# libshoal/Green-Marl

Hardware: AMD Instinct MI355X
Metric: edges/s (GTEPS) per PageRank iter, RMAT-26 (higher is better)
Workload: dtype f32; 1 GPU; pagerank RMAT-26 (V=67108864, E=1073741824), reference RMAT generator seed 1997 permute=1, d=0.85, fixed iterations; partition=1-D vertex, 1 rank(s), exchange=none, exchange_bytes_per_rank_and_step=0, exchange_packed=False, step_form=single rank, options=15

## Files before the change

green-marl_amd/csrc/gmx_pr_cold.hip:

```cpp
#pragma clang fp contract(off)

#include "gmx_internal.h"

#include <algorithm>
#include <rocprim/rocprim.hpp>

#define PRC_G 32
#define PRC_BLK_GROUPS 16
#define PRC_LDS_BYTES 131072
#define PRC_STAGE_BYTES 2048
#define PRC_LDS_LIMIT 163840
static constexpr int prc_tile_elems(int elem) { return (PRC_LDS_LIMIT - 16 * (PRC_STAGE_BYTES + 64 * elem) - 64) / elem; }
static constexpr int prc_tile_elems_classed(int elem) {
    return (PRC_LDS_LIMIT - 16 * 64 * elem - 64) / elem < 32768 ? (PRC_LDS_LIMIT - 16 * 64 * elem - 64) / elem / 8 * 8 : 32768;
}
#define PRC_THREADS 1024
#define PRC_WAVES (PRC_THREADS / 64)
#define PRC_UNROLL 4
#define PRC_PAD 0xffffu
#define PRC_END 0x8000u
#define PRC_Q1P 0
#define PRC_Q1E 64
#define PRC_Q2 128

// ... 784 lines not shown
            V4 v;
            v.x = s_tile[ids[u].x & 0x7fffu];
            v.y = s_tile[(ids[u].x >> 16) & 0x7fffu];
            v.z = s_tile[ids[u].y & 0x7fffu];
            v.w = s_tile[(ids[u].y >> 16) & 0x7fffu];
            __builtin_nontemporal_store(v, (V4*) (val + o[u]) + (lane & 7));
        }
    }
}

template <typename S, int TILE, bool CLASSED>
__global__ void __launch_bounds__(PRC_THREADS)
pr_cold_tile_kernel(const prc_item1* __restrict__ items, int n_items, unsigned int* __restrict__ queue,
                    const S* __restrict__ contrib, const int32_t* __restrict__ org, int nranks, int64_t span, int64_t slice, int64_t T,
                    const uint16_t* __restrict__ srcl, const int32_t* __restrict__ ob, S* __restrict__ val, unsigned sink_base,
                    unsigned qbase, const int32_t* __restrict__ vst) {
    __shared__ S s_tile[TILE];
    __shared__ S s_stage[PRC_WAVES][CLASSED ? 64 : PRC_STAGE_BYTES / sizeof(S) + 64];
    __shared__ int s_item;
    const int tid = threadIdx.x, lane = tid & 63;
    const int wv = __builtin_amdgcn_readfirstlane(tid >> 6);
    const unsigned sink = sink_base + (blockIdx.x * PRC_WAVES + wv) * 64 + lane;
    int loaded = -1;
    for (;;) {
        __syncthreads();
        if (tid == 0) s_item = (int) (atomicAdd(&queue[CLASSED ? PRC_Q1E : PRC_Q1P], 1u) - qbase);
        __syncthreads();
        const int it = s_item;
        if ((unsigned) it >= (unsigned) n_items) break;
        const prc_item1 d = items[it];
        if (d.tile != loaded) {
            prc_load_tile<S, TILE>(s_tile, d.tile, org, contrib, nranks, span, slice, T);
            loaded = d.tile;
            __syncthreads();
        }
        if constexpr (CLASSED) {
            const int32_t* vs = vst + ((int64_t) d.tile << PRC_CLS_BITS);
            for (int cls = PRC_CL_E1; cls <= PRC_CL_H; cls++) {
                const int32_t lo = max(d.g0, vs[cls]), hi = min(d.g1, vs[cls + 1]);
                if (lo >= hi) continue;
                const prc_item1 seg{d.tile, lo, hi, cls + 1};
                switch (cls) {
                case PRC_CL_E1: prc_class_item<S, PRC_FORM_E1>(seg, s_tile, s_stage[wv], srcl, ob, val, sink, wv, lane); break;
                case PRC_CL_E2: prc_class_item<S, PRC_FORM_E2>(seg, s_tile, s_stage[wv], srcl, ob, val, sink, wv, lane); break;
                case PRC_CL_E4: prc_class_item<S, PRC_FORM_E4>(seg, s_tile, s_stage[wv], srcl, ob, val, sink, wv, lane); break;
                case PRC_CL_E8: prc_class_item<S, PRC_FORM_E8>(seg, s_tile, s_stage[wv], srcl, ob, val, sink, wv, lane); break;
                default: prc_class_item<S, PRC_FORM_H>(seg, s_tile, s_stage[wv], srcl, ob, val, sink, wv, lane); break;
                }
            }
        } else {
            if (d.form == PRC_FORM_PAIR) prc_pair_item<S>(d, s_tile, s_stage[wv], srcl, ob, val, sink, wv, lane);
            else prc_edge_item<S>(d, s_tile, srcl, ob, val, wv, lane);
        }
    }
}

__device__ __forceinline__ unsigned long long prc_fix_hi(double v) { return (unsigned long long) (long long) (v * 0x1p62); }

template <typename S>
__device__ __forceinline__ void prc_finish_row(const pr_cold_fuse& fz, int64_t i, double sum, double& diff_acc) {
    const int32_t od = __builtin_nontemporal_load(fz.outdeg_c + i);
    const int64_t r = __builtin_nontemporal_load(fz.active + i);
    const double old = (double) __builtin_nontemporal_load((const S*) fz.rk_c + i);
    const S vs = (S) (fz.base + fz.d * sum);
    diff_acc += fabs((double) vs - old);
    __builtin_nontemporal_store(vs, (S*) fz.rk_c + i);
    __builtin_nontemporal_store(od > 0 ? (S) ((double) vs / (double) od) : (S) 0, (S*) fz.next_owned + r);
}

template <int THREADS>
__device__ __forceinline__ void prc_block_diff(double diff_acc, double* s_red, double* __restrict__ dst) {
#pragma unroll
    for (int off = 32; off > 0; off >>= 1) diff_acc += __shfl_down(diff_acc, off, 64);
    if ((threadIdx.x & 63) == 0) s_red[threadIdx.x >> 6] = diff_acc;
    __syncthreads();
    if (threadIdx.x == 0) {
        double t = 0.0;
#pragma unroll
        for (int w = 0; w < THREADS / 64; w++) t += s_red[w];
        *dst = t;
    }
}

template <typename S, int BINROWS, int LIMBS, bool FUSE>
__global__ void __launch_bounds__(PRC_THREADS)
pr_cold_accum_kernel(const prc_item2* __restrict__ items, int n_items, unsigned int* __restrict__ queue,
                     const uint16_t* __restrict__ rowl, const S* __restrict__ val, int64_t nactive, double lo_scale,
                     S* __restrict__ cold, unsigned long long* __restrict__ scratch, pr_cold_fuse fz,
                     double* __restrict__ diff_part, unsigned qbase) {
    typedef typename prc_vec4<S>::type V4;
    __shared__ unsigned long long s_acc[LIMBS * BINROWS];
    __shared__ double s_red[PRC_WAVES];
    __shared__ int s_item;
    const int tid = threadIdx.x, lane = tid & 63;
    const int wv = __builtin_amdgcn_readfirstlane(tid >> 6);
    for (;;) {
        __syncthreads();
        if (tid == 0) s_item = (int) (atomicAdd(&queue[PRC_Q2], 1u) - qbase);
#pragma unroll 4
        for (int i = tid; i < LIMBS * BINROWS; i += PRC_THREADS) s_acc[i] = 0ull;
        __syncthreads();
        const int it = s_item;
        if ((unsigned) it >= (unsigned) n_items) break;
        const prc_item2 d = items[it];
        const int npieces = (d.g1 - d.g0 + 7) >> 3;
        for (int base = 0; base < npieces; base += PRC_WAVES * PRC_UNROLL) {
            prc_u32x2 ids[PRC_UNROLL];
            V4 v[PRC_UNROLL];
            bool ok[PRC_UNROLL];
#pragma unroll
            for (int u = 0; u < PRC_UNROLL; u++) {
                const int pc = base + u * PRC_WAVES + wv;
                const int g = d.g0 + pc * 8 + (lane >> 3);
                ok[u] = pc < npieces && g < d.g1;
                if (ok[u]) {
                    const int64_t at = (int64_t) g * (PRC_G / 4) + (lane & 7);
                    ids[u] = __builtin_nontemporal_load((const prc_u32x2*) rowl + at);
                    v[u] = __builtin_nontemporal_load((const V4*) val + at);
                }
            }
#pragma unroll
            for (int u = 0; u < PRC_UNROLL; u++) {
                if (!ok[u]) continue;
                const unsigned r[4] = {ids[u].x & 0xffffu, ids[u].x >> 16, ids[u].y & 0xffffu, ids[u].y >> 16};
                const double x[4] = {(double) v[u].x, (double) v[u].y, (double) v[u].z, (double) v[u].w};
#pragma unroll
                for (int j = 0; j < 4; j++) {
                    if (r[j] == PRC_PAD) continue;
                    PRC_CHECK(r[j] < (unsigned) BINROWS && x[j] >= 0.0 && x[j] <= 1.0);
                    const unsigned long long hi = prc_fix_hi(x[j]);
                    __hip_atomic_fetch_add(&s_acc[r[j]], hi, __ATOMIC_RELAXED, __HIP_MEMORY_SCOPE_WORKGROUP);
                    if (LIMBS > 1) {
                        const double rem = x[j] - (double) (long long) hi * 0x1p-62;
                        const unsigned long long lo = (unsigned long long) (long long) (rem * 0x1p62 * lo_scale);
                        __hip_atomic_fetch_add(&s_acc[BINROWS + r[j]], lo, __ATOMIC_RELAXED, __HIP_MEMORY_SCOPE_WORKGROUP);
                    }
                }
            }
        }
        __syncthreads();
        double diff_acc = 0.0;
        if (d.slot < 0) {
            const int64_t i0 = (int64_t) d.bin * BINROWS;
#pragma unroll 4
            for (int r = tid; r < BINROWS; r += PRC_THREADS) {
                if (i0 + r >= nactive) break;
                double sum = (double) (long long) s_acc[r] * 0x1p-62;
                if (LIMBS > 1) sum += (double) (long long) s_acc[BINROWS + r] * (0x1p-62 / lo_scale);
                if (FUSE) prc_finish_row<S>(fz, i0 + r, sum, diff_acc);
                else __builtin_nontemporal_store((S) sum, cold + i0 + r);
            }
        } else {
            unsigned long long* dst = scratch + (int64_t) d.slot * (LIMBS * BINROWS);
#pragma unroll 4
            for (int i = tid; i < LIMBS * BINROWS; i += PRC_THREADS) dst[i] = s_acc[i];
        }
        if (FUSE) prc_block_diff<PRC_THREADS>(diff_acc, s_red, diff_part + it);
    }
}

template <typename S, int BINROWS, int LIMBS, bool FUSE>
__global__ void __launch_bounds__(1024)
pr_cold_reduce_kernel(const prc_item3* __restrict__ items, int64_t nactive, double lo_scale,
                      const unsigned long long* __restrict__ scratch, S* __restrict__ cold, pr_cold_fuse fz,
                      double* __restrict__ diff_part) {
    __shared__ unsigned long long s_part[LIMBS][16][64];
    const prc_item3 d = items[blockIdx.y];
    const int lane = threadIdx.x & 63, wv = threadIdx.x >> 6;
    const int r = blockIdx.x * 64 + lane;
    const int64_t i0 = (int64_t) d.bin * BINROWS;
    unsigned long long hi = 0, lo = 0;
    const unsigned long long* src = scratch + (int64_t) d.slot0 * (LIMBS * BINROWS) + r;
#pragma unroll 4
    for (int s = wv; s < d.nslots; s += 16) {
        hi += __builtin_nontemporal_load(src + (int64_t) s * (LIMBS * BINROWS));
        if (LIMBS > 1) lo += __builtin_nontemporal_load(src + (int64_t) s * (LIMBS * BINROWS) + BINROWS);
    }
    s_part[0][wv][lane] = hi;
    if (LIMBS > 1) s_part[LIMBS - 1][wv][lane] = lo;
    __syncthreads();
    if (wv == 0 && i0 + r < nactive) {
        hi = 0;
        lo = 0;
#pragma unroll
        for (int w = 0; w < 16; w++) {
            hi += s_part[0][w][lane];
            if (LIMBS > 1) lo += s_part[LIMBS - 1][w][lane];
        }
        double v = (double) (long long) hi * 0x1p-62;
        if (LIMBS > 1) v += (double) (long long) lo * (0x1p-62 / lo_scale);
        if (FUSE) {
            double diff_acc = 0.0;
            prc_finish_row<S>(fz, i0 + r, v, diff_acc);
            s_part[0][0][lane] = (unsigned long long) __double_as_longlong(diff_acc);
        } else cold[i0 + r] = (S) v;
    } else if (FUSE && wv == 0) s_part[0][0][lane] = 0ull;
    if (FUSE && wv == 0) {
        __builtin_amdgcn_wave_barrier();
        __builtin_amdgcn_s_waitcnt(0xc07f);
        __builtin_amdgcn_wave_barrier();
        if (lane == 0) {
            double t = 0.0;
            for (int l = 0; l < 64; l++) t += __longlong_as_double((long long) s_part[0][0][l]);
            diff_part[(int64_t) blockIdx.y * gridDim.x + blockIdx.x] = t;
        }
    }
}

#define PRC_FEW_SLOTS 8
template <typename S, int BINROWS, int LIMBS, bool FUSE>
__global__ void __launch_bounds__(256)
pr_cold_reduce_few_kernel(const prc_item3* __restrict__ items, int64_t nactive, double lo_scale,
                          const unsigned long long* __restrict__ scratch, S* __restrict__ cold, pr_cold_fuse fz,
                          double* __restrict__ diff_part) {
    const prc_item3 d = items[blockIdx.y];
    const int lane = threadIdx.x & 63;
    const int rg = blockIdx.x * 4 + (threadIdx.x >> 6);
    const int r = rg * 64 + lane;
    const int64_t i0 = (int64_t) d.bin * BINROWS;
    unsigned long long hi = 0, lo = 0;
    const unsigned long long* src = scratch + (int64_t) d.slot0 * (LIMBS * BINROWS) + r;
#pragma unroll 4
    for (int s = 0; s < d.nslots; s++) {
        hi += __builtin_nontemporal_load(src + (int64_t) s * (LIMBS * BINROWS));
        if (LIMBS > 1) lo += __builtin_nontemporal_load(src + (int64_t) s * (LIMBS * BINROWS) + BINROWS);
    }
    double diff_acc = 0.0;
    if (i0 + r < nactive) {
        double v = (double) (long long) hi * 0x1p-62;
        if (LIMBS > 1) v += (double) (long long) lo * (0x1p-62 / lo_scale);
        if (FUSE) prc_finish_row<S>(fz, i0 + r, v, diff_acc);
        else cold[i0 + r] = (S) v;
    }
    if (FUSE) {
        double t = 0.0;
        for (int l = 0; l < 64; l++) t += __shfl(diff_acc, l, 64);
        if (lane == 0) diff_part[(int64_t) blockIdx.y * (BINROWS / 64) + rg] = t;
    }
}

// ... 86 lines not shown
    } while (0)
#define PRC_ALLOC(buf, count)                        \
    do {                                             \
        if ((st = (buf).alloc((size_t) (count)))) goto done; \
    } while (0)

static int prc_env_int(const char* name, int dflt) {
    const char* v = getenv(name);
    return v && *v ? atoi(v) : dflt;
}

static hipError_t prc_exscan(const int32_t* in, int32_t* out, int64_t n, wbuf<char>& tmp, hipStream_t s) {
    size_t tb = 0;
    hipError_t e = rocprim::exclusive_scan(nullptr, tb, in, out, 0, (size_t) n, rocprim::plus<int32_t>(), s);
    if (e != hipSuccess) return e;
    if (tmp.n < tb) {
        tmp.release();
        if (tmp.alloc(tb)) return hipErrorOutOfMemory;
    }
    return rocprim::exclusive_scan((void*) tmp.p, tb, in, out, 0, (size_t) n, rocprim::plus<int32_t>(), s);
}

static hipError_t prc_inscan(const int32_t* in, int32_t* out, int64_t n, wbuf<char>& tmp, hipStream_t s) {
    size_t tb = 0;
    hipError_t e = rocprim::inclusive_scan(nullptr, tb, in, out, (size_t) n, rocprim::plus<int32_t>(), s);
    if (e != hipSuccess) return e;
    if (tmp.n < tb) {
        tmp.release();
        if (tmp.alloc(tb)) return hipErrorOutOfMemory;
    }
    return rocprim::inclusive_scan((void*) tmp.p, tb, in, out, (size_t) n, rocprim::plus<int32_t>(), s);
}

int pr_cold_create(const uint64_t* keys, int64_t Ec, const pr_cold_params& prm, hipStream_t s, pr_cold** outp) {
    *outp = nullptr;
    GMX_REQUIRE(prm.elem == 4 || prm.elem == 8, "pr cold: bad element size");
    GMX_REQUIRE(prm.T >= 0 && prm.T < prm.slice, "pr cold: threshold outside the rank range");
    GMX_REQUIRE(Ec < (1LL << 31) - (1LL << 27), "pr cold: %lld edges exceed the int32 stream positions", (long long) Ec);
    pr_cold* c = new pr_cold();
    c->prm = prm;
    c->Ec = Ec;
    const int64_t class_density = prc_env_int("GMX_PR_COLD_CLASS_DENSITY", 1);
    const bool all_classed = class_density == 1;
    c->tile = all_classed ? prc_tile_elems_classed(prm.elem) : prc_tile_elems(prm.elem);
    const int tile_src = c->tile - 1;
    c->limbs = prm.elem == 4 ? 1 : 2;
    c->binrows = PRC_LDS_BYTES / 8 / c->limbs;
    c->ncold = (int64_t) prm.nranks * (prm.slice - prm.T);
    c->ntiles = (c->ncold + tile_src - 1) / tile_src;
    c->nbins = (prm.nactive + c->binrows - 1) / c->binrows;
    if (c->nbins < 1) c->nbins = 1;
    const int tilebits = gmx_bits_for(c->ntiles), binbits = gmx_bits_for(c->nbins), vtbits = tilebits + PRC_CLS_BITS;
    const int64_t nvt = c->ntiles << PRC_CLS_BITS;
    const double pair_min = prc_env_int("GMX_PR_COLD_PAIR_X100", 125) / 100.0;
    int st = GMX_OK;
    gmx_tick tick("cold plan");
    gmx_ws_scope ws;
    wbuf<uint64_t> k1, k2;
    wbuf<int32_t> cflag, cincl, ps, pincl, pstart, plen, ppos, pos, endf, endpre, first, pfirst, groups, c1raw, c1, vtab, delta, counts, id, order2, groups2,
        c2s, c2, tab2, tstat;
    wbuf<uint32_t> ckey, key2, key2s;
    wbuf<uint8_t> mode;
    wbuf<char> tmp;
    uint64_t* sk = nullptr;
    std::vector<int32_t> hts, hvt, hdelta, vstart, h2;
    std::vector<uint8_t> hmode;
    std::vector<prc_item1> v1p, v1e;
    std::vector<prc_item2> v2;
    std::vector<prc_item3> v3;
    int64_t ngroups1 = 0, ngroups2 = 0, nc = 0, np = 0, pair_edges = 0, pair_tiles = 0, class_tiles = 0, class_edges = 0;
    hipDeviceProp_t prop;
    int dev = 0;
    if (vtbits + binbits > 32) {
        gmx_set_error("pr cold: %lld tiles x %lld bins do not fit the sort key", (long long) c->ntiles, (long long) c->nbins);
        st = GMX_ERR_ARG;
        goto done;
    }
    PRC_ALLOC(c->cold, (size_t) (prm.nactive ? prm.nactive : 1) * prm.elem);
    PRC_TRY(hipMemsetAsync(c->cold.p, 0, (size_t) (prm.nactive ? prm.nactive : 1) * prm.elem, s), "memset");
    PRC_ALLOC(c->queue, 3 * 64);
    PRC_TRY(hipMemsetAsync(c->queue.p, 0, 3 * 64 * sizeof(unsigned int), s), "memset");
    (void) hipGetDevice(&dev);
    PRC_TRY(hipGetDeviceProperties(&prop, dev), "hipGetDeviceProperties");
    c->grid = prop.multiProcessorCount;
    if (Ec == 0) {
        PRC_TRY(hipStreamSynchronize(s), "sync");
        *outp = c;
        return GMX_OK;
    }
    {
        PRC_ALLOC(k1, Ec);
        PRC_ALLOC(k2, Ec);
        hipLaunchKernelGGL(prc_keys_kernel, dim3(prc_grid_for(Ec)), dim3(256), 0, s, keys, Ec, prm, tile_src, c->binrows, binbits, k1.p);
        rocprim::double_buffer<uint64_t> db(k1.p, k2.p);
        size_t tb = 0;
        const unsigned end_bit = 32u + (unsigned) binbits + (unsigned) vtbits;
        PRC_TRY(rocprim::radix_sort_keys(nullptr, tb, db, (size_t) Ec, 16u, end_bit, s), "sort size");
        PRC_ALLOC(tmp, tb);
        PRC_TRY(rocprim::radix_sort_keys((void*) tmp.p, tb, db, (size_t) Ec, 16u, end_bit, s), "sort");
        PRC_TRY(hipStreamSynchronize(s), "sort sync");
        sk = db.current();
    }
    tick.mark("keys + main sort");
    PRC_ALLOC(cflag, Ec + 1);
    PRC_ALLOC(cincl, Ec + 1);
    PRC_ALLOC(ps, Ec + 1);
    PRC_ALLOC(pincl, Ec + 1);
    PRC_ALLOC(mode, c->ntiles + 1);
    PRC_ALLOC(tstat, 3 * (c->ntiles + 1));
    hmode.assign((size_t) c->ntiles + 1, PRC_TM_EDGE);
    for (int round = 0; round < 2; round++) {
        hipLaunchKernelGGL(prc_runs_kernel, dim3(prc_grid_for(Ec)), dim3(256), 0, s, (const uint64_t*) sk, Ec,
                           round ? (const uint8_t*) mode.p : (const uint8_t*) nullptr, 32 + binbits + PRC_CLS_BITS, cflag.p, ps.p);
        PRC_TRY(prc_inscan(cflag.p, cincl.p, Ec, tmp, s), "scan");
        PRC_TRY(prc_inscan(ps.p, pincl.p, Ec, tmp, s), "scan");
        {
            int32_t lastc = 0, lastp = 0;
            PRC_TRY(hipMemcpyAsync(&lastc, cincl.p + (Ec - 1), 4, hipMemcpyDeviceToHost, s), "copy");
            PRC_TRY(hipMemcpyAsync(&lastp, pincl.p + (Ec - 1), 4, hipMemcpyDeviceToHost, s), "copy");
            PRC_TRY(hipStreamSynchronize(s), "sync");
            c->ncells = nc = lastc;
            np = lastp;
        }
        if (pstart.n < (size_t) np + 1) { pstart.release(); PRC_ALLOC(pstart, np + 1); }
        hipLaunchKernelGGL(prc_pair_start_kernel, dim3(prc_grid_for(Ec + 1)), dim3(256), 0, s, (const int32_t*) ps.p, (const int32_t*) pincl.p, Ec, np, pstart.p);
        if (round == 1) break;
        hipLaunchKernelGGL(prc_tile_stats_kernel, dim3(prc_grid_for(c->ntiles + 1)), dim3(256), 0, s, (const uint64_t*) sk, Ec,
                           32 + binbits + PRC_CLS_BITS, c->ntiles, (const int32_t*) pincl.p, (const int32_t*) cincl.p, np, nc, tstat.p);
        hts.resize((size_t) 3 * (c->ntiles + 1));
        PRC_TRY(hipMemcpyAsync(hts.data(), tstat.p, sizeof(int32_t) * hts.size(), hipMemcpyDeviceToHost, s), "copy");
        PRC_TRY(hipStreamSynchronize(s), "sync");
        for (int64_t t = 0; t < c->ntiles; t++) {
            const int64_t ne = (int64_t) hts[3 * (t + 1)] - hts[3 * t], npt = (int64_t) hts[3 * (t + 1) + 1] - hts[3 * t + 1],
                          nct = (int64_t) hts[3 * (t + 1) + 2] - hts[3 * t + 2];
            hmode[t] = (npt > 0 && (double) ne >= pair_min * (double) npt) ? PRC_TM_PAIR : PRC_TM_EDGE;
            if (hmode[t] == PRC_TM_PAIR) { pair_edges += ne; pair_tiles++; }
            if (hmode[t] == PRC_TM_PAIR && class_density > 0 && ne >= class_density * nct) { hmode[t] = PRC_TM_CLASSED; class_tiles++; class_edges += ne; }
            else if (hmode[t] == PRC_TM_EDGE && all_classed && ne > 0) { hmode[t] = PRC_TM_SINGLES; class_tiles++; class_edges += ne; }
        }
        PRC_TRY(hipMemcpyAsync(mode.p, hmode.data(), hmode.size(), hipMemcpyHostToDevice, s), "copy");
        if (class_tiles == 0) continue;
        hipLaunchKernelGGL(prc_class_kernel, dim3(prc_grid_for(Ec)), dim3(256), 0, s, sk, Ec, (const int32_t*) pincl.p, (const int32_t*) pstart.p,
                           (const uint8_t*) mode.p, binbits);
        {
            uint64_t* other = sk == k1.p ? k2.p : k1.p;
            rocprim::double_buffer<uint64_t> db(sk, other);
            size_t tb = 0;
            const unsigned b0 = 32u + (unsigned) binbits, b1 = b0 + (unsigned) vtbits;
            PRC_TRY(rocprim::radix_sort_keys(nullptr, tb, db, (size_t) Ec, b0, b1, s), "sort size");
            if (tmp.n < tb) { tmp.release(); PRC_ALLOC(tmp, tb); }
            PRC_TRY(rocprim::radix_sort_keys((void*) tmp.p, tb, db, (size_t) Ec, b0, b1, s), "sort");
            PRC_TRY(hipStreamSynchronize(s), "sort sync");
            sk = db.current();
        }
    }
    if (sk == k1.p) k2.release(); else k1.release();
    tick.mark("runs, classes, class sort");
    ps.release();
    PRC_ALLOC(plen, np + 1);
    PRC_ALLOC(ppos, np + 1);
    hipLaunchKernelGGL(prc_pair_len_kernel, dim3(prc_grid_for(np + 1)), dim3(256), 0, s, (const uint64_t*) sk, (const int32_t*) pstart.p, np, binbits, plen.p);
    PRC_TRY(prc_exscan(plen.p, ppos.p, np + 1, tmp, s), "scan");
    plen.release();
    PRC_ALLOC(first, nc + 1);
    PRC_ALLOC(pfirst, nc + 1);
    PRC_ALLOC(ckey, nc + 1);
    PRC_ALLOC(groups, nc + 1);
// ... 119 lines not shown
    }
    if (prm.deg_by_id) {
        wbuf<int32_t> tmax;
        PRC_ALLOC(tmax, c->ntiles);
        PRC_TRY(hipMemsetAsync(tmax.p, 0, sizeof(int32_t) * (size_t) c->ntiles, s), "memset");
        const int64_t nids = (int64_t) prm.nranks * prm.slice;
        hipLaunchKernelGGL(prc_tile_maxdeg_kernel, dim3(prc_grid_for(nids)), dim3(256), 0, s, prm.deg_by_id, nids, prm.slice, prm.T, tile_src, tmax.p);
        c->tile_maxdeg.assign((size_t) c->ntiles, 0);
        PRC_TRY(hipMemcpyAsync(c->tile_maxdeg.data(), tmax.p, sizeof(int32_t) * (size_t) c->ntiles, hipMemcpyDeviceToHost, s), "copy");
        PRC_TRY(hipStreamSynchronize(s), "sync");
    }
    {
        const int64_t want1 = std::max<int64_t>(ngroups1 / ((int64_t) c->grid * 4), std::min<int64_t>(8192, ngroups1 / ((int64_t) c->grid * 2)));
        const int64_t want2 = ngroups2 / ((int64_t) c->grid * 2);
        const int ch1 = (int) std::min<int64_t>(262144, std::max<int64_t>(PRC_SUPER_GROUPS, prc_env_int("GMX_PR_COLD_CHUNK1", (int) std::min<int64_t>(want1, 32768)))) / PRC_SUPER_GROUPS * PRC_SUPER_GROUPS;
        const int ch2 = (int) std::min<int64_t>(32768, std::max<int64_t>(8, prc_env_int("GMX_PR_COLD_CHUNK", (int) std::min<int64_t>(std::max<int64_t>(want2, 2048), 32768)))) / 8 * 8;
        const int64_t thr2 = (int64_t) ch2 * prc_env_int("GMX_PR_COLD_SPLIT_X100", 300) / 100;
        for (int64_t t = 0; t < c->ntiles; t++) {
            const int64_t v0 = t << PRC_CLS_BITS;
            if (hmode[t] == PRC_TM_CLASSED || hmode[t] == PRC_TM_SINGLES) {
                const int32_t g0 = vstart[v0 + PRC_CL_E1], g1 = vstart[v0 + PRC_CL_H + 1];
                for (int32_t g = g0; g < g1; g += ch1) v1p.push_back({(int32_t) t, g, std::min(g1, g + ch1), PRC_FORM_TILE});
                continue;
            }
            const int32_t graw = hvt[2 * (v0 + 1) + 1] - hvt[2 * v0 + 1];
            if (graw == 0) continue;
            const int32_t g0 = vstart[v0];
            const int form = hmode[t] == PRC_TM_PAIR ? PRC_FORM_PAIR : PRC_FORM_EDGE;
            const int32_t g1 = form == PRC_FORM_PAIR ? vstart[v0 + 1] : g0 + graw;
            for (int32_t g = g0; g < g1; g += ch1) (form == PRC_FORM_EDGE ? v1e : v1p).push_back({(int32_t) t, g, std::min(g1, g + ch1), form});
        }
        PRC_ALLOC(c->vstart, vstart.size());
        PRC_TRY(hipMemcpy(c->vstart.p, vstart.data(), sizeof(int32_t) * vstart.size(), hipMemcpyHostToDevice), "copy");
        int32_t slot = 0;
        c->all_bins = true;
        for (int64_t b = 0; b < c->nbins; b++) {
            const int32_t g0 = h2[b], g1 = h2[b + 1];
            if (g1 <= g0) { c->all_bins = false; continue; }
            if (g1 - g0 <= thr2) { v2.push_back({(int32_t) b, g0, g1, -1}); continue; }
            const int32_t s0 = slot;
            for (int32_t g = g0; g < g1; g += ch2) v2.push_back({(int32_t) b, g, std::min(g1, g + ch2), slot++});
            v3.push_back({(int32_t) b, s0, slot - s0, 0});
        }
        c->n1p = (int64_t) v1p.size();
        c->n1e = (int64_t) v1e.size();
        c->n2 = (int64_t) v2.size();
        c->n3 = (int64_t) v3.size();
        c->nslots = slot;
        PRC_ALLOC(c->it1p, std::max<size_t>(1, v1p.size() + v1e.size()));
        PRC_ALLOC(c->it2, std::max<size_t>(1, v2.size()));
        PRC_ALLOC(c->it3, std::max<size_t>(1, v3.size()));
        PRC_ALLOC(c->scratch, std::max<size_t>(1, (size_t) slot * c->limbs * c->binrows));
        PRC_ALLOC(c->diffp, std::max<size_t>(1, v2.size() + v3.size() * (size_t) (c->binrows / 64)));
        PRC_TRY(hipMemset(c->diffp.p, 0, sizeof(double) * std::max<size_t>(1, v2.size() + v3.size() * (size_t) (c->binrows / 64))), "memset");
        c->h1p.swap(v1p);
        c->h1e.swap(v1e);
        c->h2.swap(v2);
        c->h3.swap(v3);
        if ((st = prc_upload_lists(c, nullptr, nullptr, 1))) goto done;
    }
    PRC_TRY(hipStreamSynchronize(s), "sync");
    tick.mark("tables, work lists");
    if (getenv("GMX_PR_DEBUG")) {
        std::vector<int64_t> bs;
        for (int64_t b = 0; b < c->nbins; b++) bs.push_back(((int64_t) h2[b + 1] - h2[b]) * PRC_G);
        std::sort(bs.begin(), bs.end());
        int64_t over[4] = {0, 0, 0, 0}, lim[4] = {131072, 262144, 524288, 1048576}, sum_over[4] = {0, 0, 0, 0};
        for (int64_t v : bs)
            for (int q = 0; q < 4; q++)
                if (v > lim[q]) { over[q]++; sum_over[q] += v; }
        fprintf(stderr, "gmx pr cold: bin items min %lld median %lld p90 %lld max %lld; bins over 128K/256K/512K/1M items: %lld/%lld/%lld/%lld holding %lld/%lld/%lld/%lld items\n",
                (long long) bs.front(), (long long) bs[bs.size() / 2], (long long) bs[bs.size() * 9 / 10], (long long) bs.back(),
                (long long) over[0], (long long) over[1], (long long) over[2], (long long) over[3], (long long) sum_over[0],
                (long long) sum_over[1], (long long) sum_over[2], (long long) sum_over[3]);
        int64_t cg[1 << PRC_CLS_BITS] = {0};
        for (int64_t v = 0; v < nvt; v++) cg[v & ((1 << PRC_CLS_BITS) - 1)] += (int64_t) vstart[v + 1] - vstart[v];
        fprintf(stderr, "gmx pr cold: T %lld, %lld edges -> %lld entries in %lld cells (%lld tiles x %lld bins); %lld pair tiles with %lld edges, of them %lld "
                "in length classes with %lld edges; groups by class generic/E1/E2/E4/E8/H %lld/%lld/%lld/%lld/%lld/%lld; %lld natural pairs -> %lld item ends -> "
                "%lld items; work items %lld + %lld / %lld / %lld, %lld slots, lo_bits %d\n", (long long) prm.T, (long long) Ec,
                (long long) c->P1, (long long) nc, (long long) c->ntiles, (long long) c->nbins, (long long) pair_tiles, (long long) pair_edges,
                (long long) class_tiles, (long long) class_edges, (long long) cg[0], (long long) cg[1], (long long) cg[2], (long long) cg[3],
                (long long) cg[4], (long long) cg[5], (long long) np, (long long) c->npairs, (long long) c->P2, (long long) c->n1p,
                (long long) c->n1e, (long long) c->n2, (long long) c->n3, (long long) c->nslots, c->lo_bits);
    }
done:
    if (st != GMX_OK) {
        delete c;
        return st;
    }
    *outp = c;
    return GMX_OK;
}

void pr_cold_free(pr_cold* c) { delete c; }

const void* pr_cold_partial(const pr_cold* c) { return c ? (const void*) c->cold.p : nullptr; }
int64_t pr_cold_edges(const pr_cold* c) { return c ? c->Ec : 0; }
int64_t pr_cold_items(const pr_cold* c) { return c ? c->P2 : 0; }

template <typename S, int TILE>
static void prc_gather_tile(pr_cold* c, const void* contrib, int k0, int k1, hipStream_t s) {
    const int64_t span = c->prm.slice - c->prm.T;
    for (int k = k0; k < k1; k++) {
        const int64_t nc = c->o1g[k] - c->o1[k], ng = c->o1[k + 1] - c->o1g[k];
        if (nc > 0) {
            const unsigned grid = (unsigned) std::min<int64_t>(c->grid, nc);
            hipLaunchKernelGGL((pr_cold_tile_kernel<S, TILE, true>), dim3(grid), dim3(PRC_THREADS), 0, s,
                               (const prc_item1*) c->it1p.p + c->o1[k], (int) nc, c->queue.p, (const S*) contrib, (const int32_t*) c->torg.p, c->prm.nranks, span,
                               c->prm.slice, c->prm.T, (const uint16_t*) c->srcl.p, (const int32_t*) c->ob.p, (S*) c->val.p, (unsigned) c->P2, c->q1c, (const int32_t*) c->vstart.p);
            c->q1c += (uint32_t) nc + grid;
        }
        if constexpr (TILE == prc_tile_elems((int) sizeof(S))) {
            if (ng > 0) {
                const unsigned grid = (unsigned) std::min<int64_t>(c->grid, ng);
                hipLaunchKernelGGL((pr_cold_tile_kernel<S, TILE, false>), dim3(grid), dim3(PRC_THREADS), 0, s,
                                   (const prc_item1*) c->it1p.p + c->o1g[k], (int) ng, c->queue.p, (const S*) contrib, (const int32_t*) c->torg.p, c->prm.nranks, span,
                                   c->prm.slice, c->prm.T, (const uint16_t*) c->srcl.p, (const int32_t*) c->ob.p, (S*) c->val.p, (unsigned) c->P2, c->q1, (const int32_t*) c->vstart.p);
                c->q1 += (uint32_t) ng + grid;
            }
        }
    }
}
template <typename S>
static void prc_gather(pr_cold* c, const void* contrib, int k0, int k1, hipStream_t s) {
    if (c->tile == prc_tile_elems_classed((int) sizeof(S))) prc_gather_tile<S, prc_tile_elems_classed((int) sizeof(S))>(c, contrib, k0, k1, s);
    else prc_gather_tile<S, prc_tile_elems((int) sizeof(S))>(c, contrib, k0, k1, s);
}

template <typename S, bool FUSE>
static void prc_accumulate(pr_cold* c, const pr_cold_fuse& fz, int q, hipStream_t s) {
    constexpr int LIMBS = sizeof(S) == 4 ? 1 : 2;
    constexpr int BINROWS = PRC_LDS_BYTES / 8 / LIMBS;
    const double lo_scale = ldexp(1.0, c->lo_bits);
    const int64_t a2 = c->o2[(size_t) q], n2 = c->o2[(size_t) q + 1] - a2;
    if (n2 > 0) {
        const unsigned grid = (unsigned) std::min<int64_t>(c->grid, n2);
        hipLaunchKernelGGL((pr_cold_accum_kernel<S, BINROWS, LIMBS, FUSE>), dim3(grid), dim3(PRC_THREADS), 0, s,
                           (const prc_item2*) c->it2.p + a2, (int) n2, c->queue.p, (const uint16_t*) c->rowl.p, (const S*) c->val.p,
                           c->prm.nactive, lo_scale, (S*) c->cold.p, c->scratch.p, fz, c->diffp.p + a2, c->q2);
        c->q2 += (uint32_t) n2 + grid;
    }
    const int64_t a3 = c->o3[(size_t) q], n3 = c->o3[(size_t) q + 1] - a3, few = c->o3few[(size_t) q];
    if (few > 0)
        hipLaunchKernelGGL((pr_cold_reduce_few_kernel<S, BINROWS, LIMBS, FUSE>), dim3(BINROWS / 256, (unsigned) few), dim3(256), 0, s,
                           (const prc_item3*) c->it3.p + a3, c->prm.nactive, lo_scale, (const unsigned long long*) c->scratch.p, (S*) c->cold.p,
                           fz, c->diffp.p + c->n2 + a3 * (BINROWS / 64));
    if (n3 > few)
        hipLaunchKernelGGL((pr_cold_reduce_kernel<S, BINROWS, LIMBS, FUSE>), dim3(BINROWS / 64, (unsigned) (n3 - few)), dim3(1024), 0, s,
                           (const prc_item3*) c->it3.p + a3 + few, c->prm.nactive, lo_scale, (const unsigned long long*) c->scratch.p, (S*) c->cold.p,
                           fz, c->diffp.p + c->n2 + (a3 + few) * (BINROWS / 64));
}

static int prc_after_launches(pr_cold* c, hipStream_t s) {
    const hipError_t e = hipGetLastError();
    if (e == hipSuccess) return GMX_OK;
    (void) hipMemsetAsync(c->queue.p, 0, 3 * 64 * sizeof(unsigned int), s);
    c->q1 = c->q1c = c->q2 = 0;
    gmx_set_error("pr cold: kernel launch failed: %s (work counters reset)", hipGetErrorString(e));
    return GMX_ERR_HIP;
}

int pr_cold_gather(pr_cold* c, const void* contrib, int cls, hipStream_t s) {
    if (!c || c->Ec == 0 || c->n2 == 0) return GMX_OK;
    const int k0 = cls < 0 ? 0 : cls, k1 = cls < 0 ? 2 : cls + 1;
    if (c->prm.elem == 4) prc_gather<float>(c, contrib, k0, k1, s);
    else prc_gather<double>(c, contrib, k0, k1, s);
// ... 49 lines not shown
```

Baseline: 748.8 GTEPS.

## Software-pipeline cold accumulation: prefetch next item and overlap drain with loads

Restructures the persistent accumulation kernel so that each block claims its next work item before finishing the current one and double-buffers the edge loads across item boundaries. The next item's first batch of loads is issued while the shared accumulators are drained to registers and written out. The per-row finish loads (outdeg, active, old rank) are batched ahead of the stores. The cross-block diff reduction is deferred by one item to save a barrier. This removes the per-item load latency bubble and extra syncs, at the cost of more register pressure and more complex control flow. It also adds an env knob for grid size and a debug dump that calls getenv without a null check.

Result: no change. 755.6 GTEPS, median of 6 (+0.9%).

```diff
diff --git a/green-marl_amd/csrc/gmx_pr_cold.hip b/green-marl_amd/csrc/gmx_pr_cold.hip
--- a/green-marl_amd/csrc/gmx_pr_cold.hip
+++ b/green-marl_amd/csrc/gmx_pr_cold.hip
@@ -890,80 +890,170 @@
     }
 }
 
+template <typename S>
+struct prc_acc_set {
+    prc_u32x2 ids[PRC_UNROLL];
+    typename prc_vec4<S>::type v[PRC_UNROLL];
+};
+
+template <typename S>
+__device__ __forceinline__ void prc_acc_load(prc_acc_set<S>& t, const prc_item2 d, const int base, const uint16_t* __restrict__ rowl,
+                                             const S* __restrict__ val, const int wv, const int lane) {
+    typedef typename prc_vec4<S>::type V4;
+#pragma unroll
+    for (int u = 0; u < PRC_UNROLL; u++) {
+        const int g = d.g0 + (base + u * PRC_WAVES + wv) * 8;
+        const unsigned at = (unsigned) (lane >> 3) * (PRC_G / 4) + (lane & 7);
+        if (g + (lane >> 3) < d.g1) {
+            t.ids[u] = __builtin_nontemporal_load((const prc_u32x2*) rowl + (int64_t) g * (PRC_G / 4) + at);
+            t.v[u] = __builtin_nontemporal_load((const V4*) val + (int64_t) g * (PRC_G / 4) + at);
+        }
+    }
+}
+
+template <typename S, int BINROWS, int LIMBS>
+__device__ __forceinline__ void prc_acc_consume(const prc_acc_set<S>& t, const prc_item2 d, const int base, unsigned long long* __restrict__ s_acc,
+                                                const double lo_scale, const int wv, const int lane) {
+#pragma unroll
+    for (int u = 0; u < PRC_UNROLL; u++) {
+        if (d.g0 + (base + u * PRC_WAVES + wv) * 8 + (lane >> 3) >= d.g1) continue;
+        const unsigned r[4] = {t.ids[u].x & 0xffffu, t.ids[u].x >> 16, t.ids[u].y & 0xffffu, t.ids[u].y >> 16};
+        const double x[4] = {(double) t.v[u].x, (double) t.v[u].y, (double) t.v[u].z, (double) t.v[u].w};
+#pragma unroll
+        for (int j = 0; j < 4; j++) {
+            if (r[j] == PRC_PAD) continue;
+            PRC_CHECK(r[j] < (unsigned) BINROWS && x[j] >= 0.0 && x[j] <= 1.0);
+            const unsigned long long hi = prc_fix_hi(x[j]);
+            __hip_atomic_fetch_add(&s_acc[r[j]], hi, __ATOMIC_RELAXED, __HIP_MEMORY_SCOPE_WORKGROUP);
+            if (LIMBS > 1) {
+                const double rem = x[j] - (double) (long long) hi * 0x1p-62;
+                const unsigned long long lo = (unsigned long long) (long long) (rem * 0x1p62 * lo_scale);
+                __hip_atomic_fetch_add(&s_acc[BINROWS + r[j]], lo, __ATOMIC_RELAXED, __HIP_MEMORY_SCOPE_WORKGROUP);
+            }
+        }
+    }
+}
+
 template <typename S, int BINROWS, int LIMBS, bool FUSE>
 __global__ void __launch_bounds__(PRC_THREADS)
 pr_cold_accum_kernel(const prc_item2* __restrict__ items, int n_items, unsigned int* __restrict__ queue,
                      const uint16_t* __restrict__ rowl, const S* __restrict__ val, int64_t nactive, double lo_scale,
                      S* __restrict__ cold, unsigned long long* __restrict__ scratch, pr_cold_fuse fz,
                      double* __restrict__ diff_part, unsigned qbase) {
-    typedef typename prc_vec4<S>::type V4;
+    constexpr int NR = BINROWS / PRC_THREADS;
+    constexpr int NA = LIMBS * NR;
+    constexpr int NB = sizeof(S) == 4 ? 8 : 4;
+    constexpr int ROUND = PRC_WAVES * PRC_UNROLL;
     __shared__ unsigned long long s_acc[LIMBS * BINROWS];
     __shared__ double s_red[PRC_WAVES];
-    __shared__ int s_item;
+    __shared__ int s_item[2];
     const int tid = threadIdx.x, lane = tid & 63;
     const int wv = __builtin_amdgcn_readfirstlane(tid >> 6);
+    if (tid == 0) s_item[0] = (int) (atomicAdd(&queue[PRC_Q2], 1u) - qbase);
+#pragma unroll 4
+    for (int i = tid; i < LIMBS * BINROWS; i += PRC_THREADS) s_acc[i] = 0ull;
+    __syncthreads();
+    int it = __builtin_amdgcn_readfirstlane(s_item[0]);
+    if ((unsigned) it >= (unsigned) n_items) return;
+    prc_item2 d = items[it];
+    prc_acc_set<S> A;
+    prc_acc_load<S>(A, d, 0, rowl, val, wv, lane);
+    int prev = -1;
     for (;;) {
+        unsigned claimed = 0;
+        bool asked = false;
+        {
+            const int npieces = (d.g1 - d.g0 + 7) >> 3;
+            int base = 0;
+            for (;;) {
+                if (!asked && base + 2 * ROUND >= npieces) {
+                    if (tid == 0) claimed = atomicAdd(&queue[PRC_Q2], 1u);
+                    asked = true;
+                }
+                prc_acc_consume<S, BINROWS, LIMBS>(A, d, base, s_acc, lo_scale, wv, lane);
+                base += ROUND;
+                if (base >= npieces) break;
+                prc_acc_load<S>(A, d, base, rowl, val, wv, lane);
+            }
+        }
+        if (tid == 0) s_item[1] = (int) (claimed - qbase);
         __syncthreads();
-        if (tid == 0) s_item = (int) (atomicAdd(&queue[PRC_Q2], 1u) - qbase);
-#pragma unroll 4
-        for (int i = tid; i < LIMBS * BINROWS; i += PRC_THREADS) s_acc[i] = 0ull;
-        __syncthreads();
-        const int it = s_item;
-        if ((unsigned) it >= (unsigned) n_items) break;
-        const prc_item2 d = items[it];
-        const int npieces = (d.g1 - d.g0 + 7) >> 3;
-        for (int base = 0; base < npieces; base += PRC_WAVES * PRC_UNROLL) {
-            prc_u32x2 ids[PRC_UNROLL];
-            V4 v[PRC_UNROLL];
-            bool ok[PRC_UNROLL];
-#pragma unroll
-            for (int u = 0; u < PRC_UNROLL; u++) {
-                const int pc = base + u * PRC_WAVES + wv;
-                const int g = d.g0 + pc * 8 + (lane >> 3);
-                ok[u] = pc < npieces && g < d.g1;
-                if (ok[u]) {
-                    const int64_t at = (int64_t) g * (PRC_G / 4) + (lane & 7);
-                    ids[u] = __builtin_nontemporal_load((const prc_u32x2*) rowl + at);
-                    v[u] = __builtin_nontemporal_load((const V4*) val + at);
-                }
+        const int nxt = __builtin_amdgcn_readfirstlane(s_item[1]);
+        const bool more = (unsigned) nxt < (unsigned) n_items;
+        prc_item2 dn = d;
+        if (more) dn = items[nxt];
+        if (FUSE && prev >= 0 && tid == 0) {
+            double t = 0.0;
+#pragma unroll
+            for (int w = 0; w < PRC_WAVES; w++) t += s_red[w];
+            diff_part[prev] = t;
+        }
+        if (more) prc_acc_load<S>(A, dn, 0, rowl, val, wv, lane);
+        const int64_t i0 = (int64_t) d.bin * BINROWS;
+        const unsigned last = (unsigned) min<int64_t>(nactive - 1 - i0, BINROWS - 1);
+        unsigned t0 = (unsigned) tid;
+        asm volatile("" : "+v"(t0));
+        int32_t od[NB], row[NB];
+        S old[NB];
+        auto row_loads = [&](const int k0) {
+#pragma unroll
+            for (int k = 0; k < NB; k++) {
+                const unsigned r = min(t0 + (k0 + k) * PRC_THREADS, last);
+                od[k] = __builtin_nontemporal_load(fz.outdeg_c + i0 + r);
+                row[k] = __builtin_nontemporal_load(fz.active + i0 + r);
+                old[k] = __builtin_nontemporal_load((const S*) fz.rk_c + i0 + r);
             }
-#pragma unroll
-            for (int u = 0; u < PRC_UNROLL; u++) {
-                if (!ok[u]) continue;
-                const unsigned r[4] = {ids[u].x & 0xffffu, ids[u].x >> 16, ids[u].y & 0xffffu, ids[u].y >> 16};
-                const double x[4] = {(double) v[u].x, (double) v[u].y, (double) v[u].z, (double) v[u].w};
-#pragma unroll
-                for (int j = 0; j < 4; j++) {
-                    if (r[j] == PRC_PAD) continue;
-                    PRC_CHECK(r[j] < (unsigned) BINROWS && x[j] >= 0.0 && x[j] <= 1.0);
-                    const unsigned long long hi = prc_fix_hi(x[j]);
-                    __hip_atomic_fetch_add(&s_acc[r[j]], hi, __ATOMIC_RELAXED, __HIP_MEMORY_SCOPE_WORKGROUP);
-                    if (LIMBS > 1) {
-                        const double rem = x[j] - (double) (long long) hi * 0x1p-62;
-                        const unsigned long long lo = (unsigned long long) (long long) (rem * 0x1p62 * lo_scale);
-                        __hip_atomic_fetch_add(&s_acc[BINROWS + r[j]], lo, __ATOMIC_RELAXED, __HIP_MEMORY_SCOPE_WORKGROUP);
-                    }
-                }
-            }
+        };
+        if (FUSE && d.slot < 0) row_loads(0);
+        unsigned long long acc[NA];
+#pragma unroll
+        for (int k = 0; k < NA; k++) {
+            acc[k] = s_acc[tid + k * PRC_THREADS];
+            s_acc[tid + k * PRC_THREADS] = 0ull;
         }
         __syncthreads();
         double diff_acc = 0.0;
         if (d.slot < 0) {
-            const int64_t i0 = (int64_t) d.bin * BINROWS;
-#pragma unroll 4
-            for (int r = tid; r < BINROWS; r += PRC_THREADS) {
-                if (i0 + r >= nactive) break;
-                double sum = (double) (long long) s_acc[r] * 0x1p-62;
-                if (LIMBS > 1) sum += (double) (long long) s_acc[BINROWS + r] * (0x1p-62 / lo_scale);
-                if (FUSE) prc_finish_row<S>(fz, i0 + r, sum, diff_acc);
-                else __builtin_nontemporal_store((S) sum, cold + i0 + r);
+#pragma unroll
+            for (int k0 = 0; k0 < NR; k0 += NB) {
+                if (FUSE && k0 > 0) row_loads(k0);
+#pragma unroll
+                for (int k = 0; k < NB; k++) {
+                    const unsigned r = t0 + (k0 + k) * PRC_THREADS;
+                    if (r > last) continue;
+                    double sum = (double) (long long) acc[k0 + k] * 0x1p-62;
+                    if (LIMBS > 1) sum += (double) (long long) acc[NR + k0 + k] * (0x1p-62 / lo_scale);
+                    if (FUSE) {
+                        const S vs = (S) (fz.base + fz.d * sum);
+                        diff_acc += fabs((double) vs - (double) old[k]);
+                        __builtin_nontemporal_store(vs, (S*) fz.rk_c + i0 + r);
+                        __builtin_nontemporal_store(od[k] > 0 ? (S) ((double) vs / (double) od[k]) : (S) 0, (S*) fz.next_owned + (int64_t) row[k]);
+                    } else __builtin_nontemporal_store((S) sum, cold + i0 + r);
+                }
             }
         } else {
-            unsigned long long* dst = scratch + (int64_t) d.slot * (LIMBS * BINROWS);
-#pragma unroll 4
-            for (int i = tid; i < LIMBS * BINROWS; i += PRC_THREADS) dst[i] = s_acc[i];
-        }
-        if (FUSE) prc_block_diff<PRC_THREADS>(diff_acc, s_red, diff_part + it);
+            unsigned long long* dst = scratch + (int64_t) d.slot * (LIMBS * BINROWS) + t0;
+#pragma unroll
+            for (int k = 0; k < NA; k++) dst[k * PRC_THREADS] = acc[k];
+        }
+        if (FUSE) {
+#pragma unroll
+            for (int off = 32; off > 0; off >>= 1) diff_acc += __shfl_down(diff_acc, off, 64);
+            if (lane == 0) s_red[wv] = diff_acc;
+            prev = it;
+        }
+        if (!more) break;
+        it = nxt;
+        d = dn;
+    }
+    if (FUSE) {
+        __syncthreads();
+        if (tid == 0) {
+            double t = 0.0;
+#pragma unroll
+            for (int w = 0; w < PRC_WAVES; w++) t += s_red[w];
+            diff_part[prev] = t;
+        }
     }
 }
 
@@ -1216,7 +1306,7 @@
     PRC_TRY(hipMemsetAsync(c->queue.p, 0, 3 * 64 * sizeof(unsigned int), s), "memset");
     (void) hipGetDevice(&dev);
     PRC_TRY(hipGetDeviceProperties(&prop, dev), "hipGetDeviceProperties");
-    c->grid = prop.multiProcessorCount;
+    c->grid = std::min(std::max(prc_env_int("GMX_PR_COLD_GRID", prop.multiProcessorCount), 1), prop.multiProcessorCount);
     if (Ec == 0) {
         PRC_TRY(hipStreamSynchronize(s), "sync");
         *outp = c;
@@ -1502,6 +1592,11 @@
                 (long long) class_tiles, (long long) class_edges, (long long) cg[0], (long long) cg[1], (long long) cg[2], (long long) cg[3],
                 (long long) cg[4], (long long) cg[5], (long long) np, (long long) c->npairs, (long long) c->P2, (long long) c->n1p,
                 (long long) c->n1e, (long long) c->n2, (long long) c->n3, (long long) c->nslots, c->lo_bits);
+        if (atoi(getenv("GMX_PR_DEBUG")) >= 3) {
+            fprintf(stderr, "gmx pr cold: phase-2 items ");
+            for (const prc_item2& w : c->h2) fputc(w.slot < 0 ? 'W' : 'c', stderr);
+            fputc('\n', stderr);
+        }
     }
 done:
     if (st != GMX_OK) {
```
